# alexeygrigorev/kubernetes-deep-learning

Measured on AMD Instinct MI355X. Metric: images/sec (whole node) + p50 latency, Xception 299x299 at 1/2/4/8 MI355X, higher is better.
Workload: dtype bf16; 1 GPU; model=Keras Xception 299x299 + clothing head (21,067,390 params), global_batch=32, image_size=299, per_gpu_batch=32, parallelism=dp1, ingress=local, egress=local, hipgraph=True, lanes=1, stages=2 (cut after block8_sepconv3)

## Files before the change

kdl/csrc/bindings_gpu.cpp:

```cpp
#include <pybind11/pybind11.h>
#include <pybind11/stl.h>

#include "kernels/launch.h"
#include "runtime/engine.h"
#include "runtime/comm.h"
#include "runtime/dp_hiploop.h"
#include "runtime/hip_backend.h"

namespace py = pybind11;
using namespace kdl;

namespace {

template <typename T>
T* P(const py::dict& d, const char* k) {
  if (!d.contains(k) || d[k].is_none()) return nullptr;
  return reinterpret_cast<T*>(d[k].cast<uintptr_t>());
}
int I(const py::dict& d, const char* k, int def = 0) {
  if (!d.contains(k) || d[k].is_none()) return def;
  return d[k].cast<int>();
}
hipStream_t S(uintptr_t s) { return reinterpret_cast<hipStream_t>(s); }

ConvGemmArgs conv_args(const py::dict& d) {
  ConvGemmArgs a{};
  a.x = P<const uint16_t>(d, "x");
  a.wp = P<const uint16_t>(d, "wp");
  a.bias = P<const float>(d, "bias");
  a.dww = P<const float>(d, "dww");
  a.dwk = P<const uint16_t>(d, "dwk");
  a.res = P<const uint16_t>(d, "res");
  a.y = P<uint16_t>(d, "y");
  a.stamps = P<unsigned long long>(d, "stamps");
  a.B = I(d, "B"); a.H = I(d, "H"); a.W = I(d, "W");
  a.OH = I(d, "OH"); a.OW = I(d, "OW"); a.M = I(d, "M");
  a.ldx = I(d, "ldx"); a.ldy = I(d, "ldy"); a.ldr = I(d, "ldr");
  a.K = I(d, "K"); a.cin = I(d, "cin", 32); a.NF = I(d, "NF");
  a.nstore = I(d, "nstore"); a.stride = I(d, "stride", 1);
  a.relu_in = I(d, "relu_in"); a.relu_out = I(d, "relu_out"); a.opad = I(d, "opad");
  a.dt = I(d, "dt");
  a.krot = I(d, "krot");
  a.ksplit = I(d, "ksplit");
  a.ws = P<float>(d, "ws");
  a.cnt = P<int>(d, "cnt");
  a.ascale = P<const float>(d, "ascale");
  a.ascale_ld = I(d, "ascale_ld");
  return a;
}
float F(const py::dict& d, const char* k, float def) {
  if (!d.contains(k) || d[k].is_none()) return def;
  return d[k].cast<float>();
}
StemArgs stem_args(const py::dict& d) {
  StemArgs a{};
  a.x = P<const void>(d, "x"); a.wp = P<const uint16_t>(d, "wp");
  a.bias = P<const float>(d, "bias"); a.y = P<uint16_t>(d, "y");
  a.B = I(d, "B"); a.H = I(d, "H"); a.W = I(d, "W");
  a.OH = I(d, "OH"); a.OW = I(d, "OW"); a.ldy = I(d, "ldy"); a.in_kind = I(d, "in_kind");
  a.KH = I(d, "KH", 3); a.KW = I(d, "KW", 3); a.stride = I(d, "stride", 2); a.pad = I(d, "pad", 0);
  a.cout = I(d, "cout", 32); a.relu = I(d, "relu", 1); a.dt = I(d, "dt");
  const char* sk[3] = {"scale0", "scale1", "scale2"};
  const char* hk[3] = {"shift0", "shift1", "shift2"};
  for (int c = 0; c < 3; ++c) { a.scale[c] = F(d, sk[c], 1.f); a.shift[c] = F(d, hk[c], 0.f); }
  a.rows = I(d, "rows", 0);
  return a;
}
GapArgs gap_args(const py::dict& d) {
  GapArgs a{};
  a.x = P<const uint16_t>(d, "x"); a.y = P<float>(d, "y"); a.yb = P<uint16_t>(d, "yb");
// ... 515 lines not shown
```

kdl/csrc/kernels/conv_gemm.hip:

```cpp
#include "common.h"
#include "launch.h"
#include "epilogue.h"

namespace kdl {

enum { MODE_PW = 0, MODE_CONV = 1, MODE_DW = 2 };

template <int MODE, int FM, int FN, int WGM, int WGN, int DT = 0>
__global__ __launch_bounds__(64 * WGM * WGN) void conv_gemm_kernel(ConvGemmArgs a) {
  using E = Elt<DT>;
  static_assert(MODE != MODE_DW || DT == 0, "the fused depthwise producer is bf16-only");
  constexpr int NW = WGM * WGN;
  constexpr int NT = 64 * NW;
  constexpr int BM = 16 * FM * WGM;
  constexpr int BN = 16 * FN * WGN;
  constexpr int AFRAGS = BM / 16;
  constexpr int STAGE = BM * 64;
  constexpr int CS = BN * 2 + 16;
  constexpr int SMEM_MAIN = 2 * STAGE;
  constexpr int SMEM_C = BM * CS;
  constexpr int SMEM = SMEM_MAIN > SMEM_C ? SMEM_MAIN : SMEM_C;
  __shared__ __attribute__((aligned(16))) uint8_t smem[SMEM];

  const int tid = threadIdx.x;
// ... 204 lines not shown
template <int MODE, int FM, int FN, int WGM, int WGN, int DT>
static hipError_t launch_cfg(const ConvGemmArgs& a, hipStream_t s) {
  constexpr int BM = 16 * FM * WGM, BN = 16 * FN * WGN;
  if ((a.NF * 16) % BN != 0) return hipErrorInvalidValue;
  const int nM = (a.M + BM - 1) / BM, nN = (a.NF * 16) / BN;
  hipLaunchKernelGGL((conv_gemm_kernel<MODE, FM, FN, WGM, WGN, DT>), dim3(nM * nN), dim3(64 * WGM * WGN), 0, s, a);
  return hipGetLastError();
}

template <int MODE, int DT = 0>
static hipError_t launch_mode(int cfg, const ConvGemmArgs& a, hipStream_t s) {
  switch (cfg) {
#define KDL_CASE(id, fm, fn, wgm, wgn) \
  case id: return launch_cfg<MODE, fm, fn, wgm, wgn, DT>(a, s);
    KDL_CONFIGS(KDL_CASE)
#undef KDL_CASE
    default: return hipErrorInvalidValue;
  }
}

hipError_t conv_gemm(int mode, int cfg, const ConvGemmArgs& a, hipStream_t s) {
  if (a.K % 32 != 0 || a.M <= 0 || a.dt < 0 || a.dt > 1) return hipErrorInvalidValue;
  if (a.ascale && cfg < STREAM_CFG_BASE && (cfg < PIPE_CFG_BASE || cfg >= SEP_CFG_BASE)) return hipErrorInvalidValue;
  if (cfg >= STREAM_CFG_BASE)
    return mode == MODE_PW && cfg <= STREAM_CFG_BASE + 1 ? gemm_stream(a, cfg == STREAM_CFG_BASE + 1, s)
                                                         : hipErrorInvalidValue;
  if (a.ksplit > 1 && (cfg < PIPE_CFG_BASE || cfg >= SEP_CFG_BASE)) return hipErrorInvalidValue;
  if (a.dt == 1) {
    if (cfg >= SEP_CFG_BASE) return hipErrorInvalidValue;
    if (cfg >= PIPE_CFG_BASE) return gemm_pipe(mode, cfg - PIPE_CFG_BASE, a, s);
    if (mode == MODE_PW) return launch_mode<MODE_PW, 1>(cfg, a, s);
    if (mode == MODE_CONV) return launch_mode<MODE_CONV, 1>(cfg, a, s);
    return hipErrorInvalidValue;
  }
  if (cfg >= C3_CFG_BASE) return mode == MODE_CONV ? conv3x3_2d(cfg - C3_CFG_BASE, a, s) : hipErrorInvalidValue;
  if (cfg >= S2D_CFG_BASE) return mode == MODE_DW ? sepconv_2d(cfg - S2D_CFG_BASE, a, s) : hipErrorInvalidValue;
  if (cfg >= SEPW_CFG_BASE) return mode == MODE_DW ? sepconv_ws(cfg - SEPW_CFG_BASE, a, s) : hipErrorInvalidValue;
  if (cfg >= SEP_CFG_BASE) return hipErrorInvalidValue;
  if (cfg >= PIPE_CFG_BASE) return gemm_pipe(mode, cfg - PIPE_CFG_BASE, a, s);
  switch (mode) {
    case MODE_PW: return launch_mode<MODE_PW>(cfg, a, s);
    case MODE_CONV: return launch_mode<MODE_CONV>(cfg, a, s);
    case MODE_DW: return launch_mode<MODE_DW>(cfg, a, s);
    default: return hipErrorInvalidValue;
  }
}
// ... 28 lines not shown
```

kdl/csrc/kernels/gemm_pipe.hip:

```cpp
#include "common.h"
#include "launch.h"
#include "epilogue.h"

namespace kdl {

__device__ __forceinline__ s16x8 pipe_ascale8(const s16x8 v, const f32x4 s0, const f32x4 s1) {
  const u32x4 u = __builtin_bit_cast(u32x4, v);
  u32x4 o;
  o[0] = pack_bf16(bf_lo(u[0]) * s0[0], bf_hi(u[0]) * s0[1]);
  o[1] = pack_bf16(bf_lo(u[1]) * s0[2], bf_hi(u[1]) * s0[3]);
  o[2] = pack_bf16(bf_lo(u[2]) * s1[0], bf_hi(u[2]) * s1[1]);
  o[3] = pack_bf16(bf_lo(u[3]) * s1[2], bf_hi(u[3]) * s1[3]);
  return __builtin_bit_cast(s16x8, o);
}

template <int N>
__device__ __forceinline__ void wait_vm_barrier() {
  asm volatile("s_waitcnt vmcnt(%0)\n\ts_barrier" ::"n"(N) : "memory");
}

template <int MODE, int FM, int FN, int WGM, int WGN, int STAGES, int KSUB, int DT = 0, bool ASC = false>
__global__ __launch_bounds__(64 * WGM * WGN) void gemm_pipe_kernel(ConvGemmArgs a) {
  using E = Elt<DT>;
  static_assert(!ASC || (MODE == 0 && DT == 0), "A-operand scales: bf16 pointwise only");
  constexpr int NW = WGM * WGN;
  constexpr int BM = 16 * FM * WGM;
  constexpr int BN = 16 * FN * WGN;
  constexpr int AF = BM / 16, BF = BN / 16;
  constexpr int FRD = AF + BF;
  constexpr int FR = FRD + (ASC ? 1 : 0);
  constexpr int L = (FR + NW - 1) / NW;
  constexpr int STAGE = FR * 1024 * KSUB;
  constexpr int CS = BN * 2 + 16;
  constexpr int SMEM_PIPE = STAGES * STAGE;
  constexpr int SMEM_C = BM * CS;
  constexpr int SMEM = SMEM_PIPE > SMEM_C ? SMEM_PIPE : SMEM_C;
  __shared__ __attribute__((aligned(16))) uint8_t smem[SMEM];

  const int tid = threadIdx.x, lane = tid & 63;
  const int wave = __builtin_amdgcn_readfirstlane(tid >> 6);
  const int wm = wave / WGN, wn = wave % WGN;
  const int nN = (a.NF * 16) / BN;
  const int OHW = a.OH * a.OW;
  constexpr bool per_img = ASC;
  const int mpi = per_img ? (OHW + BM - 1) / BM : 0;
  const int nM = per_img ? a.B * mpi : (a.M + BM - 1) / BM;
  const int S = a.ksplit > 1 ? a.ksplit : 1;
// ... 49 lines not shown
        koff_a = ((long)(tap / 3) * a.W + (tap % 3)) * a.ldx + c0;
      }
      uint8_t* base = smem + buf * STAGE + ks * FR * 1024;
#pragma unroll
      for (int i = 0; i < L; ++i) {
        const int f = min(wave + i * NW, FR - 1);
        if (f < AF) glds16(a.x + src[i] + koff_a, base + f * 1024);
        else if (!ASC || f < FRD) glds16(a.wp + src[i] + (long)k32 * 512, base + f * 1024);
        else glds16(a.ascale + src[i] + (long)k32 * 32, base + f * 1024);
      }
    }
  };

  f32x4 acc[FM][FN];
#pragma unroll
  for (int i = 0; i < FM; ++i)
#pragma unroll
    for (int j = 0; j < FN; ++j) acc[i][j] = (f32x4){0.f, 0.f, 0.f, 0.f};

#pragma unroll
  for (int p = 0; p < STAGES - 1; ++p)
    if (p < KT) issue(p, p);

  for (int t = 0; t < KT; ++t) {
    const int after = min(KT - 1, t + STAGES - 2) - t;
    if (after >= 2) wait_vm_barrier<2 * L * KSUB>();
    else if (after == 1) wait_vm_barrier<L * KSUB>();
    else wait_vm_barrier<0>();
    if (t + STAGES - 1 < KT) issue(t + STAGES - 1, (t + STAGES - 1) % STAGES);
#pragma unroll
    for (int ks = 0; ks < KSUB; ++ks) {
      if (KSUB > 1 && t * KSUB + ks >= KT32) break;
      const uint8_t* st = smem + (t % STAGES) * STAGE + ks * FR * 1024 + lane * 16;
      s16x8 af[FM], bf[FN];
#pragma unroll
      for (int i = 0; i < FM; ++i) af[i] = *(const s16x8*)(st + (wm * FM + i) * 1024);
#pragma unroll
      for (int j = 0; j < FN; ++j) bf[j] = *(const s16x8*)(st + (AF + wn * FN + j) * 1024);
      if constexpr (ASC) {
        const uint8_t* sc = st - lane * 16 + FRD * 1024 + (lane >> 4) * 32;
        const f32x4 s0 = *(const f32x4*)sc, s1 = *(const f32x4*)(sc + 16);
#pragma unroll
        for (int i = 0; i < FM; ++i) af[i] = pipe_ascale8(af[i], s0, s1);
      }
      __builtin_amdgcn_s_setprio(1);
#pragma unroll
// ... 42 lines not shown
        for (int j = 0; j < FN; ++j) {
          const float4 v = part[sp * sstride + pidx(i, j)];
          acc[i][j][0] += v.x; acc[i][j][1] += v.y; acc[i][j][2] += v.z; acc[i][j][3] += v.w;
        }
    }
  }

  const int quad = lane >> 4, col = lane & 15;
#pragma unroll
  for (int j = 0; j < FN; ++j) {
    const int nl = wn * FN * 16 + j * 16 + 4 * quad;
    const float4 bv = *(const float4*)(a.bias + n0 + nl);
#pragma unroll
    for (int i = 0; i < FM; ++i) {
      const int ml = wm * FM * 16 + i * 16 + col;
      float v0 = acc[i][j][0] + bv.x, v1 = acc[i][j][1] + bv.y;
      float v2 = acc[i][j][2] + bv.z, v3 = acc[i][j][3] + bv.w;
      if (a.relu_out == 1) {
        v0 = fmaxf(v0, 0.f); v1 = fmaxf(v1, 0.f); v2 = fmaxf(v2, 0.f); v3 = fmaxf(v3, 0.f);
      }
      *(u32x2*)(smem + ml * CS + nl * 2) = (u32x2){E::pack(v0, v1), E::pack(v2, v3)};
    }
  }
  constexpr int CPR = BN / 8;
  constexpr int NIT = (BM * CPR + 64 * NW - 1) / (64 * NW);
  u32x4 rres[NIT];
  if (a.res) {
#pragma unroll
    for (int it = 0; it < NIT; ++it) {
      const int c = tid + it * 64 * NW, r = c / CPR, cc = c - r * CPR;
      const int m = min(m0 + r, a.M - 1), n = min(n0 + cc * 8, a.nstore - 8);
      rres[it] = c < BM * CPR ? *(const u32x4*)(a.res + (long)m * a.ldr + n) : (u32x4){0u, 0u, 0u, 0u};
    }
  }
  __syncthreads();
#pragma unroll
  for (int it = 0; it < NIT; ++it) {
    const int c = tid + it * 64 * NW, r = c / CPR, cc = c - r * CPR;
    const int m = m0 + r, n = n0 + cc * 8;
    if (c < BM * CPR && m < mend && n < a.nstore)
      epi_store_r<DT>(a, m, n, *(const u32x4*)(smem + r * CS + cc * 16), rres[it]);
  }
}

#define KDL_PIPE_CONFIGS(X) \
  X(0, 4, 4, 2, 2, 4, 1)    \
  X(1, 2, 4, 2, 2, 4, 1)    \
  X(2, 4, 2, 2, 2, 4, 1)    \
  X(3, 2, 2, 2, 2, 4, 1)    \
  X(4, 8, 2, 1, 4, 4, 1)    \
// ... 7 lines not shown
  X(12, 2, 6, 2, 4, 3, 1)   \
  X(13, 4, 2, 2, 4, 3, 1)   \
  X(14, 3, 3, 2, 4, 2, 2)   \
  X(15, 6, 3, 2, 4, 2, 2)   \
  X(16, 4, 2, 2, 4, 2, 2)   \
  X(17, 4, 4, 2, 2, 3, 2)   \
  X(18, 3, 3, 2, 4, 3, 2)   \
  X(19, 4, 4, 2, 2, 2, 4)   \
  X(20, 2, 4, 2, 2, 3, 2)   \
  X(21, 4, 2, 2, 2, 3, 2)   \
  X(22, 6, 3, 2, 4, 5, 1)   \
  X(23, 3, 6, 2, 4, 5, 1)   \
  X(24, 3, 3, 2, 4, 6, 1)   \
  X(25, 4, 2, 2, 4, 6, 1)   \
  X(26, 6, 3, 2, 4, 3, 2)    \
  X(27, 5, 2, 2, 4, 3, 2)   \
  X(28, 5, 3, 2, 4, 3, 2)   \
  X(29, 5, 4, 2, 4, 2, 2)   \
  X(30, 5, 2, 2, 4, 4, 1)   \
  X(45, 5, 2, 2, 4, 3, 1)   \
  X(46, 5, 3, 2, 4, 3, 1)   \
  X(47, 5, 4, 2, 4, 3, 1)

template <int MODE, int FM, int FN, int WGM, int WGN, int ST, int KS, int DT = 0, bool ASC = false>
static hipError_t launch_pipe_cfg(const ConvGemmArgs& a, hipStream_t s) {
  constexpr int BM = 16 * FM * WGM, BN = 16 * FN * WGN;
  if ((a.NF * 16) % BN != 0) return hipErrorInvalidValue;
  constexpr bool per_img = ASC;
  if (per_img && (a.M != a.B * a.OH * a.OW || a.B <= 0)) return hipErrorInvalidValue;
  if (ASC && (!a.ascale || a.ascale_ld < a.K || a.ascale_ld % 4 != 0)) return hipErrorInvalidValue;
  const int nM = per_img ? a.B * ((a.OH * a.OW + BM - 1) / BM) : (a.M + BM - 1) / BM, nN = (a.NF * 16) / BN;
  const int S = a.ksplit > 1 ? a.ksplit : 1;
  if (S > 1 && ((a.K / 32) % S != 0 || !a.ws || !a.cnt || per_img || S > 16)) return hipErrorInvalidValue;
  hipLaunchKernelGGL((gemm_pipe_kernel<MODE, FM, FN, WGM, WGN, ST, KS, DT, ASC>), dim3(nM * nN * S),
                     dim3(64 * WGM * WGN), 0, s, a);
  return hipGetLastError();
}

template <int MODE, int DT, bool ASC = false>
static hipError_t launch_pipe_mode(int cfg, const ConvGemmArgs& a, hipStream_t s) {
  switch (cfg) {
#define KDL_PCASE(id, fm, fn, wgm, wgn, st, ks) \
  case id: return launch_pipe_cfg<MODE, fm, fn, wgm, wgn, st, ks, DT, ASC>(a, s);
    KDL_PIPE_CONFIGS(KDL_PCASE)
#undef KDL_PCASE
    default: return hipErrorInvalidValue;
  }
}

hipError_t gemm_pipe(int mode, int cfg, const ConvGemmArgs& args, hipStream_t s) {
  if (args.K % 32 != 0 || args.M <= 0 || args.dt < 0 || args.dt > 1) return hipErrorInvalidValue;
  static const int env_krot = [] { const char* e = getenv("KDL_PIPE_KROT"); return e ? atoi(e) : -1; }();
  ConvGemmArgs a = args;
  if (env_krot >= 0) a.krot = env_krot;
  if (a.ascale) {
    if (mode != 0 || a.dt != 0 || a.ksplit > 1) return hipErrorInvalidValue;
    return launch_pipe_mode<0, 0, true>(cfg, a, s);
  }
  if (mode == 0) return a.dt ? launch_pipe_mode<0, 1>(cfg, a, s) : launch_pipe_mode<0, 0>(cfg, a, s);
  if (mode == 1) return a.dt ? launch_pipe_mode<1, 1>(cfg, a, s) : launch_pipe_mode<1, 0>(cfg, a, s);
  return hipErrorInvalidValue;
}

int gemm_pipe_config(int cfg, int* bm, int* bn, int* threads) {
  switch (cfg) {
#define KDL_PINFO(id, fm, fn, wgm, wgn, st, ks) \
  case id: *bm = 16 * fm * wgm; *bn = 16 * fn * wgn; *threads = 64 * wgm * wgn; return 0;
    KDL_PIPE_CONFIGS(KDL_PINFO)
#undef KDL_PINFO
    default: return -1;
  }
}

}
```

kdl/csrc/kernels/launch.h:

```cpp
#pragma once
#include <hip/hip_runtime.h>
#include <stdint.h>

namespace kdl {

struct ConvGemmArgs {
  const uint16_t* x;
  const uint16_t* wp;
  const float* bias;
  const float* dww;
  const uint16_t* dwk;
  const uint16_t* res;
  uint16_t* y;
  int B, H, W;
  int OH, OW;
  int M;
  int ldx, ldy, ldr;
  int K;
  int cin;
  int NF;
  int nstore;
  int stride;
  int relu_in;
  int relu_out;
  unsigned long long* stamps;
  int opad;
  int dt;
  int krot;
  int ksplit;
  float* ws;
  int* cnt;
  const float* ascale;
  int ascale_ld;
};

constexpr int PIPE_CFG_BASE = 16;
constexpr int SEP_CFG_BASE = 64;
constexpr int SEPW_CFG_BASE = 120;
hipError_t sepconv_ws(int cfg, const ConvGemmArgs& a, hipStream_t s);
int sepconv_ws_config(int cfg, int* bm, int* bn, int* threads);
int sepconv_ws_fits(int cfg, int W);

struct EntryBlockArgs {
  const uint16_t* x;
  uint16_t* y;
  const uint16_t* w1;
  const float* b1;
  const float* dw1;
  const uint16_t* w2;
  const float* b2;
  const float* dw2;
  const uint16_t* dwk1;
  const uint16_t* dwk2;
  const uint16_t* wr;
  const float* br;
  int B, H, W, OH, OW, ldx, ldy;
// ... 220 lines not shown
```

kdl/engine/stages.py:

```python
from __future__ import annotations

import ctypes
import os
from dataclasses import dataclass

import torch


def _cu_mask(k: int, shares: list, n_cu: int = 256) -> list[int]:
    bounds, acc = [], 0.0
    for f in shares:
        acc += f
        bounds.append(round(acc * 20))
    lo = 0 if k == 0 else bounds[k - 1]
    hi = bounds[k]
    words = [0] * ((n_cu + 31) // 32)
    for i in range(n_cu):
        if lo <= i % 20 < hi:
            words[i // 32] |= 1 << (i % 32)
    return words


def cu_masked_stream(device, words: list[int]) -> torch.cuda.ExternalStream:
    hip = ctypes.CDLL("libamdhip64.so")
    hip.hipExtStreamCreateWithCUMask.argtypes = [ctypes.POINTER(ctypes.c_void_p), ctypes.c_uint32,
                                                  ctypes.POINTER(ctypes.c_uint32)]
    arr = (ctypes.c_uint32 * len(words))(*words)
    ptr = ctypes.c_void_p()
    with torch.cuda.device(device):
        err = hip.hipExtStreamCreateWithCUMask(ctypes.byref(ptr), len(words), arr)
    if err != 0:
        raise RuntimeError(f"hipExtStreamCreateWithCUMask failed ({err})")
    return torch.cuda.ExternalStream(ptr.value, device=device)


@dataclass
class StagePlan:
    ranges: list
    remaps: list
    boundary: list
    wait_for: list
    aliases: dict


def plan_stages(steps, split_after, scratch=()) -> StagePlan:
    cuts = split_after.split(",") if isinstance(split_after, str) else list(split_after)
    names = [s.name for s in steps]
    for c in cuts:
        if c not in names:
            raise ValueError(f"no step {c!r}; steps: {names}")
    bounds = [0] + sorted(names.index(c) + 1 for c in cuts) + [len(names)]
    ranges = [(lo, hi) for lo, hi in zip(bounds, bounds[1:]) if hi > lo]
    K = len(ranges)
    stage = [k for k, (lo, hi) in enumerate(ranges) for _ in range(lo, hi)]
    last_write: dict = {}
    reads = []
    readers: dict = {}
    for i, st in enumerate(steps):
        r = {}
        for nm in (st.src, st.res):
            if nm and nm not in ("input", "logits"):
                w = last_write.get(nm, -1)
                r[nm] = w
                if w >= 0:
                    readers[w] = max(readers.get(w, stage[w]), stage[i])
        reads.append(r)
        if st.dst and st.dst not in ("input", "logits") and st.src != st.dst:
            last_write[st.dst] = i
    touched: dict = {}
    for i, st in enumerate(steps):
# ... 167 lines not shown
```

kdl/engine/xception.py:

```python
from __future__ import annotations

import os
from pathlib import Path

import torch

from ..models import xception as X
from ..models.layers import tf_same_pad
from ..ops import _lib
from ..ops.conv import MODE_CONV, MODE_DW, MODE_PW, ConvGemmLayer, Geometry, conv_weights_nk
from ..ops.pack import bn_scale_shift, pack_fragments, round_up, rowrun_weights
from .base import EngineBase, Step


class XceptionEngine(EngineBase):
    model_name = "xception"

    def __init__(self, params: dict, max_batch: int = 32, device: str | torch.device = "cuda",
                 in_kind: str = "u8", head: X.Head = X.DEFAULT_HEAD, buckets=None,
                 tune_file: str | Path | None = None):
        super().__init__(device, max_batch, buckets)
        self.in_kind = in_kind
        self.head = head
        eb = os.environ.get("KDL_ENTRY_BLOCK", "2:15,3")
        spec = "2,3" if eb == "1" else ("" if eb == "0" else eb)
        self.fused_blocks = {}
        for v in filter(None, (x.strip() for x in spec.split(","))):
            blk, _, cfg = v.partition(":")
            self.fused_blocks[int(blk)] = int(cfg) if cfg else None
        self.size = X.INPUT_SIZE
        self.shapes: dict[str, tuple[int, int, int]] = {}
        self._build(params)
        self._alloc()
        if tune_file and Path(tune_file).exists():
            self.load_tuning(tune_file)

    def _build(self, p: dict) -> None:
        dev = self.device
        S = self.size
        st = X.SPEC
        c1 = st[0].main[0]
        s, t = bn_scale_shift(p, c1.bn)
        w = p[f"{c1.name}/kernel"].double().reshape(27, 32).t() * s[:, None]
        if self.in_kind == "u8":
            bias = t - w.sum(1)
            w = w / 127.5
        else:
            bias = t
        oh1 = (S - 3) // 2 + 1
        self.stem_rows = self.in_kind == "u8" and os.environ.get("KDL_STEM_ROWS", "1") != "0"
        if self.stem_rows:
            self.stem_wp = pack_fragments(rowrun_weights(w, 3, 9, 16), 2, 2).to(dev).contiguous()
        else:
            self.stem_wp = pack_fragments(w, 2, 1).to(dev).contiguous()
        self.stem_bias = bias.float().to(dev)
        self.steps.append(Step("stem", c1.name, src="input", dst="stem1", geom=(S, S, oh1, oh1)))
        self.shapes["stem1"] = (oh1, oh1, 32)
        c2 = st[0].main[1]
        s, t = bn_scale_shift(p, c2.bn)
        w = conv_weights_nk(p[f"{c2.name}/kernel"], 32) * s[:, None]
        lay = ConvGemmLayer(c2.name, MODE_CONV, w, t, cin_pad=32, n=64, relu_out=True, device=dev)
        h = oh1 - 2
        self.steps.append(Step("conv", c2.name, lay, "stem1", "stem2", geom=(oh1, oh1, h, h)))
        self.shapes["stem2"] = (h, h, 64)
        cur, H = "stem2", h
        for bi, blk in enumerate(st[1:], start=1):
            if blk.kind in ("entry", "exit"):
                rc = blk.res_conv
                oh = (H - 1) // 2 + 1
                rname = f"{rc.name}_out"
                lay = self._pw(p, rc, dev)
                _, pt, _ = tf_same_pad(H, 3, 2)
                out = f"block{bi + 1}_out"
                if bi + 1 in self.fused_blocks:
                    from ..ops.entry_block import EntryBlock
                    s1, s2 = (self._sep(p, op, dev) for op in blk.main)
                    g = os.environ.get("KDL_ENTRY_GRID")
                    fb = EntryBlock(f"block{bi + 1}", s1, s2, lay, cfg=self.fused_blocks[bi + 1], device=dev,
                                    grid=int(g) if g else None)
                    self.steps.append(Step("block", f"block{bi + 1}", src=cur, dst=out, geom=(H, H, oh, oh),
                                           extra=dict(eb=fb)))
                    self.shapes[out] = (oh, oh, s2.ldy)
                    cur, H = out, oh
                    continue
                self.steps.append(Step("conv", rc.name, lay, cur, rname, geom=(H, H, oh, oh)))
                self.shapes[rname] = (oh, oh, lay.ldy)
                y = cur
                for op in blk.main:
                    lay = self._sep(p, op, dev)
                    dst = f"{op.name}_out"
                    self.steps.append(Step("conv", op.name, lay, y, dst, geom=(H, H, H, H)))
                    self.shapes[dst] = (H, H, lay.ldy)
                    y = dst
                C = self.shapes[y][2]
                self.steps.append(Step("pool", f"block{bi + 1}_pool", src=y, dst=out, res=rname,
                                       geom=(H, H, oh, oh), extra=dict(pad=pt, C=C)))
                self.shapes[out] = (oh, oh, C)
                cur, H = out, oh
            elif blk.kind == "middle":
                y = cur
                for k, op in enumerate(blk.main):
                    lay = self._sep(p, op, dev)
                    dst = f"{op.name}_out"
                    res = cur if k == len(blk.main) - 1 else None
                    self.steps.append(Step("conv", op.name, lay, y, dst, res=res, geom=(H, H, H, H)))
                    self.shapes[dst] = (H, H, lay.ldy)
                    y = dst
                cur = y
            else:
                for op in blk.main:
                    lay = self._sep(p, op, dev)
                    dst = f"{op.name}_out"
                    self.steps.append(Step("conv", op.name, lay, cur, dst, geom=(H, H, H, H)))
                    self.shapes[dst] = (H, H, lay.ldy)
                    cur = dst
        hd = self.head
        self.w1 = p[f"{hd.hidden}/kernel"].float().t().contiguous().to(dev)
        self.b1 = p[f"{hd.hidden}/bias"].float().to(dev)
        self.w2 = p[f"{hd.out}/kernel"].float().contiguous().to(dev)
        self.b2 = p[f"{hd.out}/bias"].float().to(dev)
        self.steps.append(Step("head", "head", src=cur, dst="logits", geom=(H, H, 1, 1)))
        self.feat_buf = cur
        self._hoist_relus()

    def _hoist_relus(self) -> None:
        uses: dict[str, int] = {}
        for st in self.steps:
            for b in (st.src, st.res):
                if b:
                    uses[b] = uses.get(b, 0) + 1
        for a, b in zip(self.steps, self.steps[1:]):
            if (a.kind == "conv" and b.kind == "conv" and b.src == a.dst and uses.get(a.dst) == 1
                    and a.res is None and a.layer.relu_out == 0 and b.layer.mode == MODE_DW and b.layer.relu_in):
                a.layer.relu_out, b.layer.relu_in = 1, False

    @staticmethod
    def _pw(p, rc, dev) -> ConvGemmLayer:
        s, t = bn_scale_shift(p, rc.bn)
        cin_pad = round_up(rc.cin, 32)
        w = torch.zeros(rc.cout, cin_pad, dtype=torch.float64)
        w[:, :rc.cin] = p[f"{rc.name}/kernel"].double()[0, 0].t() * s[:, None]
        return ConvGemmLayer(rc.name, MODE_PW, w, t, cin_pad=cin_pad, n=rc.cout, stride=2, device=dev)

    @staticmethod
    def _sep(p, op, dev) -> ConvGemmLayer:
        s, t = bn_scale_shift(p, op.bn)
        cin_pad = round_up(op.cin, 32)
        w = torch.zeros(op.cout, cin_pad, dtype=torch.float64)
        w[:, :op.cin] = p[f"{op.name}/pointwise_kernel"].double()[0, 0].t() * s[:, None]
        dww = torch.zeros(9, cin_pad, dtype=torch.float32)
        dww[:, :op.cin] = p[f"{op.name}/depthwise_kernel"].float()[:, :, :, 0].reshape(9, op.cin)
        return ConvGemmLayer(op.name, MODE_DW, w, t, cin_pad=cin_pad, n=op.cout, dww=dww,
                             relu_in=op.relu_in, relu_out=op.relu_out, device=dev,
                             ksplit=(2, 3, 4) if op.cout >= 1536 else ())

    def _alloc(self) -> None:
        B, S, dev = self.max_batch, self.size, self.device
        if self.in_kind == "u8":
            self.inp = torch.zeros((B, S, S, 3), dtype=torch.uint8, device=dev)
        else:
            self.inp = torch.zeros((B, S, S, 3), dtype=torch.float32, device=dev)
        self.bufs: dict[str, torch.Tensor] = {}
        for name, (h, w, c) in self.shapes.items():
            self.bufs[name] = torch.zeros(B * h * w * c, dtype=torch.bfloat16, device=dev)
        self.logits = torch.zeros((B, self.head.classes), dtype=torch.float32, device=dev)
# ... 29 lines not shown
        elif step.kind == "conv":
            self._emit_conv(prog, step, b)
        elif step.kind == "pool":
            prog.add_pool_add(step.name, dict(x=self._ptr(step.src), res=self._ptr(step.res),
                                              y=self._ptr(step.dst), B=b, H=H, W=W, OH=OH, OW=OW,
                                              C=step.extra["C"], pad_top=step.extra["pad"],
                                              pad_left=step.extra["pad"]))
        elif step.kind == "block":
            step.extra["eb"].emit(prog, self._ptr(step.src), self._ptr(step.dst), b, H, W)
        elif step.kind == "head":
            hd = self.head
            prog.add_head(step.name, dict(x=self._ptr(step.src), w1=_lib.ptr(self.w1),
                                          b1=_lib.ptr(self.b1), w2=_lib.ptr(self.w2),
                                          b2=_lib.ptr(self.b2), out=self._ptr("logits"),
                                          feat=_lib.ptr(self.head_feat), hid=_lib.ptr(self.head_hid),
                                          B=b, HW=H * W, ldx=self.shapes[step.src][2],
                                          F=hd.features, H1=hd.hidden_units, NC=hd.classes))

    def _emit_conv(self, prog, step: Step, b: int, split=None, cfg=None) -> None:
        H, W, OH, OW = step.geom
        step.layer.emit(prog, self._ptr(step.src), self._ptr(step.dst), Geometry(b, H, W, OH, OW),
                        res=self._ptr(step.res) if step.res else None, ldx=self.shapes[step.src][2],
                        ldr=self.shapes[step.res][2] if step.res else None, tmp=self._ptr("__dwtmp"),
                        split=split, cfg=cfg)

    def flops_per_image(self) -> float:
        return 2 * 8.356e9
```

kdl/ops/conv.py:

```python
from __future__ import annotations

from dataclasses import dataclass

import torch

from . import _lib
from .pack import pack_fragments, pad_vec, round_up

MODE_PW, MODE_CONV, MODE_DW = 0, 1, 2

PIPE_BASE = 16
CONFIGS = {0: (2, 2, 2, 2), 1: (4, 2, 2, 2), 2: (2, 4, 2, 2), 3: (4, 4, 2, 2), 4: (4, 6, 1, 8),
           5: (2, 12, 1, 4), 6: (4, 4, 1, 4), 7: (2, 6, 1, 8), 8: (8, 2, 1, 4), 9: (4, 2, 1, 4),
           16: (4, 4, 2, 2), 17: (2, 4, 2, 2), 18: (4, 2, 2, 2), 19: (2, 2, 2, 2),
           20: (8, 2, 1, 4), 21: (4, 4, 1, 4), 22: (4, 8, 2, 2), 23: (8, 4, 1, 4),
           24: (3, 6, 2, 4), 25: (6, 3, 2, 4), 26: (3, 3, 2, 4), 27: (4, 4, 2, 2),
           28: (2, 6, 2, 4), 29: (4, 2, 2, 4), 30: (3, 3, 2, 4), 31: (6, 3, 2, 4),
           32: (4, 2, 2, 4), 33: (4, 4, 2, 2), 34: (3, 3, 2, 4), 35: (4, 4, 2, 2),
           36: (2, 4, 2, 2), 37: (4, 2, 2, 2), 38: (6, 3, 2, 4), 39: (3, 6, 2, 4),
           40: (3, 3, 2, 4), 41: (4, 2, 2, 4), 42: (6, 3, 2, 4),
           43: (5, 2, 2, 4), 44: (5, 3, 2, 4), 45: (5, 4, 2, 4), 46: (5, 2, 2, 4),
           61: (5, 2, 2, 4), 62: (5, 3, 2, 4), 63: (5, 4, 2, 4),
           120: (6, 6, 1, 4), 121: (6, 6, 1, 4), 122: (6, 6, 1, 4), 123: (6, 6, 1, 4), 124: (6, 3, 1, 4),
           125: (4, 6, 1, 4), 126: (6, 6, 1, 4), 127: (6, 6, 1, 4),
# ... 10 lines not shown
           184: (3, 2, 2, 4), 185: (2, 2, 2, 4), 186: (2, 4, 2, 4), 187: (4, 2, 2, 4), 188: (3, 2, 2, 4),
           189: (2, 4, 2, 4), 190: (2, 2, 2, 4), 191: (2, 2, 2, 4), 192: (3, 2, 2, 4),
           200: (2, 2, 2, 4), 201: (4, 2, 2, 4), 202: (3, 2, 2, 4), 203: (2, 4, 2, 4), 204: (4, 2, 2, 4),
           208: (2, 2, 4, 2), 209: (1, 2, 4, 2), 210: (2, 2, 4, 2), 211: (3, 2, 4, 2),
           212: (2, 2, 4, 2), 213: (1, 2, 4, 2), 214: (2, 2, 4, 2), 215: (2, 4, 4, 1)}
S2DP = {184: (4, 6, 16), 185: (4, 4, 16), 186: (3, 4, 16), 187: (4, 8, 16), 188: (6, 6, 16), 189: (4, 4, 16),
        190: (8, 4, 16), 191: (11, 4, 16), 192: (7, 6, 16)}
S2DW = {200: (4, 4, 16), 201: (4, 8, 16), 202: (4, 6, 16), 203: (4, 4, 16), 204: (6, 8, 16)}
SEP_BASE = 64
SEPW_BASE = 120
S2D_BASE = 160
C3_BASE = 208
S2D_MIN_W = 64
SEPW_XB = {120: 9, 121: 9, 122: 11, 123: 16, 124: 9, 125: 8, 126: 9, 127: 9,
           135: 15, 136: 11, 137: 15, 140: 8, 141: 8, 142: 8,
           143: 9, 144: 11, 145: 16, 146: 8, 147: 9,
           128: 9, 129: 9, 130: 9, 131: 9, 132: 9, 133: 9, 148: 9, 149: 11, 156: 16, 157: 8, 158: 9}
SPLITK_BASE = 2000
STREAM_BASE = 3000
STREAM_NT = 3001
STREAM_IDS = (STREAM_BASE, STREAM_NT)
STREAM_SHAPES = frozenset([(1, 2), (2, 2), (1, 12), (6, 4), (2, 18), (9, 4), (9, 6), (3, 30), (15, 6)])
STREAM_SHAPES_F16 = frozenset([(2, 4), (2, 16), (8, 4), (8, 8)])
ABLATION_IDS = frozenset([127, 147, 128, 129, 130, 131, 132, 133])


def s2dp_smem(cfg: int, K: int) -> int:
    st, th, tw = S2DP[cfg] if cfg in S2DP else S2DW[cfg]
    bm, bn = cfg_tile(cfg)
    ipp = ((th + 2) * (tw + 2) + 1 + 63) // 64
    kt = K // 32
    if cfg in S2DW:
        return kt * (bn // 16) * 1024 + kt * 1024 + st * 4 * ipp * 1024 + 2 * (bm // 16) * 1024
    return kt * (bn // 16) * 1024 + kt * 1024 + st * 4 * ipp * 1024 + 2 * (bm // 16) * 1024 + bm * (bn * 2 + 16) + 1024


def config_applicable(cfg: int, W: int | None, K: int | None = None, n: int | None = None) -> bool:
    if cfg >= C3_BASE:
        return (K is None or K == 288) and (n is None or round_up(n, cfg_tile(cfg)[1]) == cfg_tile(cfg)[1])
    if cfg < SEP_BASE or W is None:
        return True
    if cfg in S2DP or cfg in S2DW:
        return (W >= S2D_MIN_W and (K is None or s2dp_smem(cfg, K) <= 160 * 1024)
                and (n is None or round_up(n, cfg_tile(cfg)[1]) == cfg_tile(cfg)[1]))
    if cfg >= S2D_BASE:
        return W >= S2D_MIN_W
# ... 44 lines not shown
            return c
    return cands[0]


@dataclass
class Geometry:
    B: int
    H: int
    W: int
    OH: int
    OW: int

    @property
    def M(self) -> int:
        return self.B * self.OH * self.OW


class ConvGemmLayer:

    def __init__(self, name: str, mode: int, w_nk: torch.Tensor, bias: torch.Tensor, *,
                 cin_pad: int, n: int, stride: int = 1, dww: torch.Tensor | None = None,
                 relu_in: bool = False, relu_out: bool | int = False, device="cuda",
                 candidates: list[int] | None = None, dtype: torch.dtype = torch.bfloat16,
                 ksplit: tuple = ()):
        assert dtype in (torch.bfloat16, torch.float16), dtype
        assert dtype == torch.bfloat16 or mode != MODE_DW, "fused separable convs are bf16-only"
        self.dtype, self.dt = dtype, int(dtype == torch.float16)
        self.name, self.mode, self.n = name, mode, n
        self.cin_pad, self.stride = cin_pad, stride
        self.relu_in, self.relu_out = relu_in, int(relu_out)
        self.K = w_nk.shape[1]
        assert self.K % 32 == 0, (name, self.K)
        self.ldy = round_up(n, 32)
        self.candidates = candidates if candidates is not None else candidate_configs(n, mode=mode)
        self.nf_max = max(round_up(n, cfg_tile(c)[1]) // 16 for c in self.candidates)
        self.cfg = default_config(mode, n, 0) if candidates is None else self.candidates[0]
        if self.cfg not in self.candidates:
            self.cfg = self.candidates[0]
        self.wp = pack_fragments(w_nk, self.nf_max, self.K // 32, dtype).to(device).contiguous()
        self.bias = pad_vec(bias, self.nf_max * 16).to(device)
        self.dww = None
        self.dwk = None
        self.krot = 0
        if mode == MODE_DW:
            assert dww is not None and dww.shape == (9, cin_pad)
            self.dww = dww.float().contiguous().to(device)
            self.dwk = pack_dw_entries(dww).to(device)
        self.w_ref = w_nk.to(dtype).float()
        self.ksplit = tuple(ksplit)
        assert not self.ksplit or mode in (MODE_PW, MODE_CONV, MODE_DW), (name, "split-K: LDS-DMA GEMM lowerings only")
        self._splitk_bufs: tuple | None = None
        self.split = False

    def variants(self, W: int | None = None) -> list[tuple[bool, int]]:
        skv = [(False, splitk_id(sk, c)) for sk in self.ksplit for c in self.candidates
               if PIPE_BASE <= c < SEP_BASE and cfg_tile(c)[0] <= 160 and (self.K // 32) % sk == 0]
        if self.mode == MODE_CONV:
            return [(False, c) for c in self.candidates
                    if c < SEP_BASE or (c >= C3_BASE and self.stride == 1 and config_applicable(c, W, self.K, self.n))] + skv
        if self.mode != MODE_DW:
            return ([(False, c) for c in self.candidates if c < SEP_BASE] + skv
                    + ([(False, c) for c in STREAM_IDS] if self.stream_ok() else []))
        return ([(False, c) for c in self.candidates
                 if (c < PIPE_BASE or c >= SEP_BASE) and config_applicable(c, W, self.K, self.n)]
                + [(True, c) for c in self.candidates if c < SEP_BASE] + [(True, c) for _, c in skv])

    def stream_ok(self, res: bool = False) -> bool:
        if res and self.ldy > 288:
            return False
        shapes = STREAM_SHAPES if self.dt == 0 else STREAM_SHAPES_F16
        return (self.mode == MODE_PW and self.stride == 1 and not self.relu_in
                and self.relu_out != 3 and (self.K // 32, self.ldy // 16) in shapes
                and self.nf_max * 16 >= self.ldy)

    def dw_args(self, x: int, tmp: int, g: Geometry, ldx: int | None = None) -> dict:
        assert (ldx or self.cin_pad) == self.cin_pad
        return dict(x=x, w=_lib.ptr(self.dww), y=tmp, B=g.B, H=g.H, W=g.W, C=self.cin_pad,
                    relu_in=int(self.relu_in))

    def emit(self, prog, x: int, y: int, g: Geometry, res: int | None = None, ldx: int | None = None,
             ldr: int | None = None, tmp: int | None = None, split: bool | None = None,
             cfg: int | None = None, opad: int = 0,
             ascale: tuple[int, int] | None = None) -> None:
        split = self.split if split is None else split
        cfg = self.cfg if cfg is None else cfg
        C = _lib.lib()
        if self.mode == MODE_DW and split:
            assert tmp is not None, "split separable conv needs a scratch buffer"
            da = self.dw_args(x, tmp, g, ldx)
            if is_splitk(cfg):
                sk, cfg = splitk_parts(cfg)
                ga = self.args(tmp, y, g, res, ldx=self.cin_pad, ldr=ldr, cfg=cfg, opad=opad)
                ws, cnt = self._splitk_workspace(sk, cfg, g.M)
                ga.update(ksplit=sk, ws=_lib.ptr(ws), cnt=_lib.ptr(cnt))
            else:
                ga = self.args(tmp, y, g, res, ldx=self.cin_pad, ldr=ldr, cfg=cfg, opad=opad)
            if prog is None:
                s = _lib.stream_ptr()
                C.dw3x3(da, s)
                C.conv_gemm(MODE_PW, cfg, ga, s)
            else:
                prog.add_dw(self.name + "/dw", da)
                prog.add_conv_gemm(self.name, MODE_PW, cfg, ga)
            return
        if is_splitk(cfg):
            sk, cfg = splitk_parts(cfg)
            assert ascale is None and (self.K // 32) % sk == 0, (self.name, sk)
            ga = self.args(x, y, g, res, ldx=ldx, ldr=ldr, cfg=cfg, opad=opad)
            ws, cnt = self._splitk_workspace(sk, cfg, g.M)
            ga.update(ksplit=sk, ws=_lib.ptr(ws), cnt=_lib.ptr(cnt))
            if prog is None:
                C.conv_gemm(self.mode, cfg, ga, _lib.stream_ptr())
            else:
                prog.add_conv_gemm(self.name, self.mode, cfg, ga)
            return
        ga = self.args(x, y, g, res, ldx=ldx, ldr=ldr, cfg=cfg, opad=opad)
        if ascale:
            assert (PIPE_BASE <= cfg < SEP_BASE or cfg in STREAM_IDS) and self.mode == MODE_PW and \
                self.dt == 0, \
                "A-operand channel scales ride the bf16 pointwise LDS-DMA pipelined or streaming GEMM"
            ga.update(ascale=ascale[0], ascale_ld=ascale[1])
        if prog is None:
            C.conv_gemm(self.mode, cfg, ga, _lib.stream_ptr())
        else:
            prog.add_conv_gemm(self.name, self.mode, cfg, ga)

    def _splitk_workspace(self, ksplit: int, cfg: int, M: int):
        bm, bn = cfg_tile(cfg)
        tiles = -(-M // bm) * (self.nf(cfg) * 16 // bn)
        need_ws, need_cnt = ksplit * tiles * bm * bn, tiles
        cur = self._splitk_bufs
        if cur is None or cur[0].numel() < need_ws or cur[1].numel() < need_cnt:
            dev = self.wp.device
            n_ws = max(need_ws, cur[0].numel() if cur else 0)
            n_cnt = max(need_cnt, cur[1].numel() if cur else 0)
            self._splitk_bufs = (torch.zeros(n_ws, dtype=torch.float32, device=dev),
                                 torch.zeros(n_cnt, dtype=torch.int32, device=dev))
            self._splitk_old = getattr(self, "_splitk_old", []) + ([cur] if cur else [])
        return self._splitk_bufs

    def nf(self, cfg: int | None = None) -> int:
        cfg = self.cfg if cfg is None else cfg
        return round_up(self.n, cfg_tile(cfg)[1]) // 16

    def args(self, x: int, y: int, g: Geometry, res: int | None = None, ldx: int | None = None,
             ldr: int | None = None, cfg: int | None = None, opad: int = 0) -> dict:
        return dict(x=x, wp=_lib.ptr(self.wp), bias=_lib.ptr(self.bias),
                    dww=_lib.ptr(self.dww), dwk=_lib.ptr(self.dwk), res=res, y=y,
                    B=g.B, H=g.H, W=g.W, OH=g.OH, OW=g.OW, M=g.M,
                    ldx=ldx if ldx is not None else self.cin_pad, ldy=self.ldy,
                    ldr=ldr if ldr is not None else self.ldy,
                    K=self.K, cin=self.cin_pad, NF=self.nf(cfg), nstore=self.ldy,
                    stride=self.stride, relu_in=int(self.relu_in), relu_out=int(self.relu_out),
                    opad=int(opad), dt=self.dt, krot=int(self.krot))

    def launch(self, x: torch.Tensor, y: torch.Tensor, g: Geometry, res: torch.Tensor | None = None,
               cfg: int | None = None, split: bool = False, tmp: torch.Tensor | None = None,
               opad: int = 0) -> None:
        self.check(x, y, g, res, opad)
        if split:
            if tmp is None:
                tmp = torch.empty(g.M * self.cin_pad, dtype=torch.bfloat16, device=x.device)
            assert tmp.numel() >= g.M * self.cin_pad
        self.emit(None, _lib.ptr(x), _lib.ptr(y), g, _lib.ptr(res), tmp=_lib.ptr(tmp), split=split, cfg=cfg,
                  opad=opad)

    def check(self, x, y, g: Geometry, res=None, opad: int = 0) -> None:
        assert x.dtype == self.dtype and y.dtype == self.dtype, (x.dtype, y.dtype, self.dtype)
        assert x.is_contiguous() and y.is_contiguous()
        assert x.numel() >= g.B * g.H * g.W * self.cin_pad, (self.name, x.shape)
        assert y.numel() >= g.B * (g.OH + 2 * opad) * (g.OW + 2 * opad) * self.ldy, (self.name, y.shape)
        if self.mode == MODE_DW:
            assert g.OH == g.H and g.OW == g.W
        elif self.mode == MODE_CONV:
            assert g.OH == (g.H - 3) // self.stride + 1 and g.OW == (g.W - 3) // self.stride + 1
        else:
            assert g.OH == (g.H - 1) // self.stride + 1 and g.OW == (g.W - 1) // self.stride + 1
        if res is not None:
            assert res.dtype == self.dtype and res.numel() >= g.M * self.ldy


def pack_dw_entries(dww: torch.Tensor) -> torch.Tensor:
    C = dww.shape[1]
    w = torch.cat([dww.float(), torch.zeros(1, C)], 0)
    w = w.view(5, 2, C // 32, 2, 16)
    e = w.permute(2, 3, 4, 1, 0)
    e = torch.cat([e, torch.zeros(*e.shape[:-1], 3)], -1)
    return e.to(torch.bfloat16).contiguous()


def conv_weights_nk(kernel_hwio: torch.Tensor, cin_pad: int) -> torch.Tensor:
    kh, kw, cin, cout = kernel_hwio.shape
    w = torch.zeros(kh * kw, cin_pad, cout, dtype=torch.float64)
    w[:, :cin, :] = kernel_hwio.double().reshape(kh * kw, cin, cout)
    return w.reshape(kh * kw * cin_pad, cout).t().contiguous()
```

Before: 25240 images/s.

## Fuse exit/entry-block maxpool into the strided residual 1x1 conv epilogue

Adds a POOL variant of the pipelined GEMM kernel that computes the 3x3 stride-2 max-pool of the main-branch output directly in registers before the K-loop and adds it as the residual. This removes the separate pool kernel and the intermediate write and read of the residual conv output for non-fused entry/exit blocks, enabled by default via KDL_EXIT_TAIL. In exchange the pooled residual does 9 gathered loads per output vector up front, which raises register pressure, and the layer is restricted to a small set of pipe configs. Stage-cut names are remapped through an alias so existing split points still resolve.

After: 25370 images/s, median of 6. Within noise of the previous version (+0.5%).

```diff
diff --git a/kdl/csrc/bindings_gpu.cpp b/kdl/csrc/bindings_gpu.cpp
--- a/kdl/csrc/bindings_gpu.cpp
+++ b/kdl/csrc/bindings_gpu.cpp
@@ -46,6 +46,8 @@
   a.cnt = P<int>(d, "cnt");
   a.ascale = P<const float>(d, "ascale");
   a.ascale_ld = I(d, "ascale_ld");
+  a.res_pool = I(d, "res_pool");
+  a.res_pad = I(d, "res_pad");
   return a;
 }
 float F(const py::dict& d, const char* k, float def) {
diff --git a/kdl/csrc/kernels/conv_gemm.hip b/kdl/csrc/kernels/conv_gemm.hip
--- a/kdl/csrc/kernels/conv_gemm.hip
+++ b/kdl/csrc/kernels/conv_gemm.hip
@@ -250,6 +250,7 @@
 hipError_t conv_gemm(int mode, int cfg, const ConvGemmArgs& a, hipStream_t s) {
   if (a.K % 32 != 0 || a.M <= 0 || a.dt < 0 || a.dt > 1) return hipErrorInvalidValue;
   if (a.ascale && cfg < STREAM_CFG_BASE && (cfg < PIPE_CFG_BASE || cfg >= SEP_CFG_BASE)) return hipErrorInvalidValue;
+  if (a.res_pool && (cfg < PIPE_CFG_BASE || cfg >= SEP_CFG_BASE)) return hipErrorInvalidValue;
   if (cfg >= STREAM_CFG_BASE)
     return mode == MODE_PW && cfg <= STREAM_CFG_BASE + 1 ? gemm_stream(a, cfg == STREAM_CFG_BASE + 1, s)
                                                          : hipErrorInvalidValue;
diff --git a/kdl/csrc/kernels/gemm_pipe.hip b/kdl/csrc/kernels/gemm_pipe.hip
--- a/kdl/csrc/kernels/gemm_pipe.hip
+++ b/kdl/csrc/kernels/gemm_pipe.hip
@@ -19,10 +19,12 @@
   asm volatile("s_waitcnt vmcnt(%0)\n\ts_barrier" ::"n"(N) : "memory");
 }
 
-template <int MODE, int FM, int FN, int WGM, int WGN, int STAGES, int KSUB, int DT = 0, bool ASC = false>
+template <int MODE, int FM, int FN, int WGM, int WGN, int STAGES, int KSUB, int DT = 0, bool ASC = false,
+          bool POOL = false>
 __global__ __launch_bounds__(64 * WGM * WGN) void gemm_pipe_kernel(ConvGemmArgs a) {
   using E = Elt<DT>;
   static_assert(!ASC || (MODE == 0 && DT == 0), "A-operand scales: bf16 pointwise only");
+  static_assert(!POOL || (MODE == 0 && DT == 0 && !ASC), "pooled residual: bf16 pointwise only");
   constexpr int NW = WGM * WGN;
   constexpr int BM = 16 * FM * WGM;
   constexpr int BN = 16 * FN * WGN;
@@ -118,6 +120,47 @@
   for (int p = 0; p < STAGES - 1; ++p)
     if (p < KT) issue(p, p);
 
+  constexpr int CPR = BN / 8;
+  constexpr int NIT = (BM * CPR + 64 * NW - 1) / (64 * NW);
+  u32x4 rres[NIT];
+  auto pool_window = [&](int it) {
+    const int c = tid + it * 64 * NW, r = c / CPR, cc = c - r * CPR;
+    const int m = min(m0 + r, a.M - 1), n = min(n0 + cc * 8, a.nstore - 8);
+    const int b = m / OHW, rem = m - b * OHW;
+    const int oh = rem / a.OW, ow = rem - oh * a.OW;
+    const int ih0 = 2 * oh - a.res_pad, iw0 = 2 * ow - a.res_pad;
+    const uint16_t* rb = a.res + (long)b * a.H * a.W * a.ldr + n;
+    u32x4 v[9];
+#pragma unroll
+    for (int dy = 0; dy < 3; ++dy) {
+      const int ih = min(max(ih0 + dy, 0), a.H - 1);
+#pragma unroll
+      for (int dx = 0; dx < 3; ++dx) {
+        const int iw = min(max(iw0 + dx, 0), a.W - 1);
+        v[dy * 3 + dx] = *(const u32x4*)(rb + (long)(ih * a.W + iw) * a.ldr);
+      }
+    }
+    float mx[8];
+#pragma unroll
+    for (int d = 0; d < 8; ++d) mx[d] = -INFINITY;
+#pragma unroll
+    for (int t = 0; t < 9; ++t)
+#pragma unroll
+      for (int d = 0; d < 4; ++d) {
+        mx[2 * d] = fmaxf(mx[2 * d], bf_lo(v[t][d]));
+        mx[2 * d + 1] = fmaxf(mx[2 * d + 1], bf_hi(v[t][d]));
+      }
+    return (u32x4){pack_bf16(mx[0], mx[1]), pack_bf16(mx[2], mx[3]), pack_bf16(mx[4], mx[5]),
+                   pack_bf16(mx[6], mx[7])};
+  };
+  if constexpr (POOL) {
+#pragma unroll
+    for (int it = 0; it < NIT; ++it) {
+      rres[it] = pool_window(it);
+      asm volatile("" : "+v"(rres[it]));
+    }
+  }
+
   for (int t = 0; t < KT; ++t) {
     const int after = min(KT - 1, t + STAGES - 2) - t;
     if (after >= 2) wait_vm_barrier<2 * L * KSUB>();
@@ -206,10 +249,7 @@
       *(u32x2*)(smem + ml * CS + nl * 2) = (u32x2){E::pack(v0, v1), E::pack(v2, v3)};
     }
   }
-  constexpr int CPR = BN / 8;
-  constexpr int NIT = (BM * CPR + 64 * NW - 1) / (64 * NW);
-  u32x4 rres[NIT];
-  if (a.res) {
+  if (!POOL && a.res) {
 #pragma unroll
     for (int it = 0; it < NIT; ++it) {
       const int c = tid + it * 64 * NW, r = c / CPR, cc = c - r * CPR;
@@ -263,7 +303,15 @@
   X(46, 5, 3, 2, 4, 3, 1)   \
   X(47, 5, 4, 2, 4, 3, 1)
 
-template <int MODE, int FM, int FN, int WGM, int WGN, int ST, int KS, int DT = 0, bool ASC = false>
+#define KDL_PIPE_POOL_CONFIGS(X) \
+  X(1, 2, 4, 2, 2, 4, 1)         \
+  X(2, 4, 2, 2, 2, 4, 1)         \
+  X(3, 2, 2, 2, 2, 4, 1)         \
+  X(10, 3, 3, 2, 4, 3, 1)        \
+  X(13, 4, 2, 2, 4, 3, 1)        \
+  X(20, 2, 4, 2, 2, 3, 2)
+
+template <int MODE, int FM, int FN, int WGM, int WGN, int ST, int KS, int DT = 0, bool ASC = false, bool POOL = false>
 static hipError_t launch_pipe_cfg(const ConvGemmArgs& a, hipStream_t s) {
   constexpr int BM = 16 * FM * WGM, BN = 16 * FN * WGN;
   if ((a.NF * 16) % BN != 0) return hipErrorInvalidValue;
@@ -273,7 +321,7 @@
   const int nM = per_img ? a.B * ((a.OH * a.OW + BM - 1) / BM) : (a.M + BM - 1) / BM, nN = (a.NF * 16) / BN;
   const int S = a.ksplit > 1 ? a.ksplit : 1;
   if (S > 1 && ((a.K / 32) % S != 0 || !a.ws || !a.cnt || per_img || S > 16)) return hipErrorInvalidValue;
-  hipLaunchKernelGGL((gemm_pipe_kernel<MODE, FM, FN, WGM, WGN, ST, KS, DT, ASC>), dim3(nM * nN * S),
+  hipLaunchKernelGGL((gemm_pipe_kernel<MODE, FM, FN, WGM, WGN, ST, KS, DT, ASC, POOL>), dim3(nM * nN * S),
                      dim3(64 * WGM * WGN), 0, s, a);
   return hipGetLastError();
 }
@@ -289,11 +337,29 @@
   }
 }
 
+static hipError_t launch_pipe_pool(int cfg, const ConvGemmArgs& a, hipStream_t s) {
+  switch (cfg) {
+#define KDL_PPCASE(id, fm, fn, wgm, wgn, st, ks) \
+  case id: return launch_pipe_cfg<0, fm, fn, wgm, wgn, st, ks, 0, false, true>(a, s);
+    KDL_PIPE_POOL_CONFIGS(KDL_PPCASE)
+#undef KDL_PPCASE
+    default: return hipErrorInvalidValue;
+  }
+}
+
 hipError_t gemm_pipe(int mode, int cfg, const ConvGemmArgs& args, hipStream_t s) {
   if (args.K % 32 != 0 || args.M <= 0 || args.dt < 0 || args.dt > 1) return hipErrorInvalidValue;
   static const int env_krot = [] { const char* e = getenv("KDL_PIPE_KROT"); return e ? atoi(e) : -1; }();
   ConvGemmArgs a = args;
   if (env_krot >= 0) a.krot = env_krot;
+  if (a.res_pool) {
+    if (mode != 0 || a.dt != 0 || a.ksplit > 1 || a.ascale || !a.res || a.res_pool != 1) return hipErrorInvalidValue;
+    if (a.stride != 2 || a.res_pad < 0 || a.res_pad > 1 || a.B <= 0 || a.M != a.B * a.OH * a.OW ||
+        a.OH != (a.H - 1) / 2 + 1 || a.OW != (a.W - 1) / 2 + 1 || 2 * a.OH - a.res_pad > a.H ||
+        2 * a.OW - a.res_pad > a.W || a.ldr < a.nstore || a.ldr % 8 != 0 || a.nstore < 8)
+      return hipErrorInvalidValue;
+    return launch_pipe_pool(cfg, a, s);
+  }
   if (a.ascale) {
     if (mode != 0 || a.dt != 0 || a.ksplit > 1) return hipErrorInvalidValue;
     return launch_pipe_mode<0, 0, true>(cfg, a, s);
diff --git a/kdl/csrc/kernels/launch.h b/kdl/csrc/kernels/launch.h
--- a/kdl/csrc/kernels/launch.h
+++ b/kdl/csrc/kernels/launch.h
@@ -32,6 +32,8 @@
   int* cnt;
   const float* ascale;
   int ascale_ld;
+  int res_pool;
+  int res_pad;
 };
 
 constexpr int PIPE_CFG_BASE = 16;
diff --git a/kdl/engine/stages.py b/kdl/engine/stages.py
--- a/kdl/engine/stages.py
+++ b/kdl/engine/stages.py
@@ -46,6 +46,8 @@
 def plan_stages(steps, split_after, scratch=()) -> StagePlan:
     cuts = split_after.split(",") if isinstance(split_after, str) else list(split_after)
     names = [s.name for s in steps]
+    aka = {a: s.name for s in steps for a in s.extra.get("aka", ()) if a not in names}
+    cuts = [aka.get(c, c) for c in cuts]
     for c in cuts:
         if c not in names:
             raise ValueError(f"no step {c!r}; steps: {names}")
diff --git a/kdl/engine/xception.py b/kdl/engine/xception.py
--- a/kdl/engine/xception.py
+++ b/kdl/engine/xception.py
@@ -15,6 +15,7 @@
 
 class XceptionEngine(EngineBase):
     model_name = "xception"
+    exit_tail = False
 
     def __init__(self, params: dict, max_batch: int = 32, device: str | torch.device = "cuda",
                  in_kind: str = "u8", head: X.Head = X.DEFAULT_HEAD, buckets=None,
@@ -28,6 +29,7 @@
         for v in filter(None, (x.strip() for x in spec.split(","))):
             blk, _, cfg = v.partition(":")
             self.fused_blocks[int(blk)] = int(cfg) if cfg else None
+        self.exit_tail = os.environ.get("KDL_EXIT_TAIL", "1") != "0"
         self.size = X.INPUT_SIZE
         self.shapes: dict[str, tuple[int, int, int]] = {}
         self._build(params)
@@ -69,10 +71,11 @@
                 rc = blk.res_conv
                 oh = (H - 1) // 2 + 1
                 rname = f"{rc.name}_out"
-                lay = self._pw(p, rc, dev)
+                fused = bi + 1 in self.fused_blocks
+                lay = self._pw(p, rc, dev, res_pool=self.exit_tail and not fused)
                 _, pt, _ = tf_same_pad(H, 3, 2)
                 out = f"block{bi + 1}_out"
-                if bi + 1 in self.fused_blocks:
+                if fused:
                     from ..ops.entry_block import EntryBlock
                     s1, s2 = (self._sep(p, op, dev) for op in blk.main)
                     g = os.environ.get("KDL_ENTRY_GRID")
@@ -83,18 +86,25 @@
                     self.shapes[out] = (oh, oh, s2.ldy)
                     cur, H = out, oh
                     continue
-                self.steps.append(Step("conv", rc.name, lay, cur, rname, geom=(H, H, oh, oh)))
-                self.shapes[rname] = (oh, oh, lay.ldy)
+                if not self.exit_tail:
+                    self.steps.append(Step("conv", rc.name, lay, cur, rname, geom=(H, H, oh, oh)))
+                    self.shapes[rname] = (oh, oh, lay.ldy)
                 y = cur
                 for op in blk.main:
-                    lay = self._sep(p, op, dev)
+                    sl = self._sep(p, op, dev)
                     dst = f"{op.name}_out"
-                    self.steps.append(Step("conv", op.name, lay, y, dst, geom=(H, H, H, H)))
-                    self.shapes[dst] = (H, H, lay.ldy)
+                    self.steps.append(Step("conv", op.name, sl, y, dst, geom=(H, H, H, H)))
+                    self.shapes[dst] = (H, H, sl.ldy)
                     y = dst
                 C = self.shapes[y][2]
-                self.steps.append(Step("pool", f"block{bi + 1}_pool", src=y, dst=out, res=rname,
-                                       geom=(H, H, oh, oh), extra=dict(pad=pt, C=C)))
+                if self.exit_tail:
+                    assert C == lay.ldy, (rc.name, C, lay.ldy)
+                    self.steps.append(Step("conv", rc.name, lay, src=cur, res=y, dst=out,
+                                           geom=(H, H, oh, oh),
+                                           extra=dict(pool_pad=pt, aka=(f"block{bi + 1}_pool",))))
+                else:
+                    self.steps.append(Step("pool", f"block{bi + 1}_pool", src=y, dst=out, res=rname,
+                                           geom=(H, H, oh, oh), extra=dict(pad=pt, C=C)))
                 self.shapes[out] = (oh, oh, C)
                 cur, H = out, oh
             elif blk.kind == "middle":
@@ -135,12 +145,13 @@
                 a.layer.relu_out, b.layer.relu_in = 1, False
 
     @staticmethod
-    def _pw(p, rc, dev) -> ConvGemmLayer:
+    def _pw(p, rc, dev, res_pool: bool = False) -> ConvGemmLayer:
         s, t = bn_scale_shift(p, rc.bn)
         cin_pad = round_up(rc.cin, 32)
         w = torch.zeros(rc.cout, cin_pad, dtype=torch.float64)
         w[:, :rc.cin] = p[f"{rc.name}/kernel"].double()[0, 0].t() * s[:, None]
-        return ConvGemmLayer(rc.name, MODE_PW, w, t, cin_pad=cin_pad, n=rc.cout, stride=2, device=dev)
+        return ConvGemmLayer(rc.name, MODE_PW, w, t, cin_pad=cin_pad, n=rc.cout, stride=2, device=dev,
+                             res_pool=res_pool)
 
     @staticmethod
     def _sep(p, op, dev) -> ConvGemmLayer:
@@ -216,7 +227,7 @@
         step.layer.emit(prog, self._ptr(step.src), self._ptr(step.dst), Geometry(b, H, W, OH, OW),
                         res=self._ptr(step.res) if step.res else None, ldx=self.shapes[step.src][2],
                         ldr=self.shapes[step.res][2] if step.res else None, tmp=self._ptr("__dwtmp"),
-                        split=split, cfg=cfg)
+                        split=split, cfg=cfg, pool_pad=step.extra.get("pool_pad"))
 
     def flops_per_image(self) -> float:
         return 2 * 8.356e9
diff --git a/kdl/ops/conv.py b/kdl/ops/conv.py
--- a/kdl/ops/conv.py
+++ b/kdl/ops/conv.py
@@ -56,6 +56,7 @@
 STREAM_IDS = (STREAM_BASE, STREAM_NT)
 STREAM_SHAPES = frozenset([(1, 2), (2, 2), (1, 12), (6, 4), (2, 18), (9, 4), (9, 6), (3, 30), (15, 6)])
 STREAM_SHAPES_F16 = frozenset([(2, 4), (2, 16), (8, 4), (8, 8)])
+POOL_IDS = frozenset([17, 18, 19, 26, 29, 36])
 ABLATION_IDS = frozenset([127, 147, 128, 129, 130, 131, 132, 133])
 
 
@@ -146,7 +147,7 @@
                  cin_pad: int, n: int, stride: int = 1, dww: torch.Tensor | None = None,
                  relu_in: bool = False, relu_out: bool | int = False, device="cuda",
                  candidates: list[int] | None = None, dtype: torch.dtype = torch.bfloat16,
-                 ksplit: tuple = ()):
+                 ksplit: tuple = (), res_pool: bool = False):
         assert dtype in (torch.bfloat16, torch.float16), dtype
         assert dtype == torch.bfloat16 or mode != MODE_DW, "fused separable convs are bf16-only"
         self.dtype, self.dt = dtype, int(dtype == torch.float16)
@@ -157,8 +158,15 @@
         assert self.K % 32 == 0, (name, self.K)
         self.ldy = round_up(n, 32)
         self.candidates = candidates if candidates is not None else candidate_configs(n, mode=mode)
+        self.res_pool = bool(res_pool)
+        if self.res_pool:
+            assert mode == MODE_PW and stride == 2 and self.dt == 0 and not ksplit, (name, "pooled residual")
+            self.candidates = [c for c in self.candidates if c in POOL_IDS]
+            assert self.candidates, (name, "no pooled-residual config fits")
         self.nf_max = max(round_up(n, cfg_tile(c)[1]) // 16 for c in self.candidates)
         self.cfg = default_config(mode, n, 0) if candidates is None else self.candidates[0]
+        if self.res_pool and candidates is None:
+            self.cfg = next((c for c in (17, 18, 19) if c in self.candidates), self.candidates[0])
         if self.cfg not in self.candidates:
             self.cfg = self.candidates[0]
         self.wp = pack_fragments(w_nk, self.nf_max, self.K // 32, dtype).to(device).contiguous()
@@ -182,6 +190,8 @@
         if self.mode == MODE_CONV:
             return [(False, c) for c in self.candidates
                     if c < SEP_BASE or (c >= C3_BASE and self.stride == 1 and config_applicable(c, W, self.K, self.n))] + skv
+        if self.res_pool:
+            return [(False, c) for c in self.candidates]
         if self.mode != MODE_DW:
             return ([(False, c) for c in self.candidates if c < SEP_BASE] + skv
                     + ([(False, c) for c in STREAM_IDS] if self.stream_ok() else []))
@@ -205,7 +215,7 @@
     def emit(self, prog, x: int, y: int, g: Geometry, res: int | None = None, ldx: int | None = None,
              ldr: int | None = None, tmp: int | None = None, split: bool | None = None,
              cfg: int | None = None, opad: int = 0,
-             ascale: tuple[int, int] | None = None) -> None:
+             ascale: tuple[int, int] | None = None, pool_pad: int | None = None) -> None:
         split = self.split if split is None else split
         cfg = self.cfg if cfg is None else cfg
         C = _lib.lib()
@@ -229,7 +239,7 @@
             return
         if is_splitk(cfg):
             sk, cfg = splitk_parts(cfg)
-            assert ascale is None and (self.K // 32) % sk == 0, (self.name, sk)
+            assert ascale is None and pool_pad is None and (self.K // 32) % sk == 0, (self.name, sk)
             ga = self.args(x, y, g, res, ldx=ldx, ldr=ldr, cfg=cfg, opad=opad)
             ws, cnt = self._splitk_workspace(sk, cfg, g.M)
             ga.update(ksplit=sk, ws=_lib.ptr(ws), cnt=_lib.ptr(cnt))
@@ -239,6 +249,9 @@
                 prog.add_conv_gemm(self.name, self.mode, cfg, ga)
             return
         ga = self.args(x, y, g, res, ldx=ldx, ldr=ldr, cfg=cfg, opad=opad)
+        if pool_pad is not None:
+            assert cfg in POOL_IDS and res is not None and not ascale, (self.name, cfg, "pooled residual")
+            ga.update(res_pool=1, res_pad=int(pool_pad))
         if ascale:
             assert (PIPE_BASE <= cfg < SEP_BASE or cfg in STREAM_IDS) and self.mode == MODE_PW and \
                 self.dt == 0, \
@@ -280,16 +293,16 @@
 
     def launch(self, x: torch.Tensor, y: torch.Tensor, g: Geometry, res: torch.Tensor | None = None,
                cfg: int | None = None, split: bool = False, tmp: torch.Tensor | None = None,
-               opad: int = 0) -> None:
-        self.check(x, y, g, res, opad)
+               opad: int = 0, pool_pad: int | None = None) -> None:
+        self.check(x, y, g, res, opad, pool_pad)
         if split:
             if tmp is None:
                 tmp = torch.empty(g.M * self.cin_pad, dtype=torch.bfloat16, device=x.device)
             assert tmp.numel() >= g.M * self.cin_pad
         self.emit(None, _lib.ptr(x), _lib.ptr(y), g, _lib.ptr(res), tmp=_lib.ptr(tmp), split=split, cfg=cfg,
-                  opad=opad)
-
-    def check(self, x, y, g: Geometry, res=None, opad: int = 0) -> None:
+                  opad=opad, pool_pad=pool_pad)
+
+    def check(self, x, y, g: Geometry, res=None, opad: int = 0, pool_pad: int | None = None) -> None:
         assert x.dtype == self.dtype and y.dtype == self.dtype, (x.dtype, y.dtype, self.dtype)
         assert x.is_contiguous() and y.is_contiguous()
         assert x.numel() >= g.B * g.H * g.W * self.cin_pad, (self.name, x.shape)
@@ -301,7 +314,8 @@
         else:
             assert g.OH == (g.H - 1) // self.stride + 1 and g.OW == (g.W - 1) // self.stride + 1
         if res is not None:
-            assert res.dtype == self.dtype and res.numel() >= g.M * self.ldy
+            rows = g.M if pool_pad is None else g.B * g.H * g.W
+            assert res.dtype == self.dtype and res.numel() >= rows * self.ldy
 
 
 def pack_dw_entries(dww: torch.Tensor) -> torch.Tensor:
```
